# arkiven4/glow-tts

Hardware: AMD Instinct MI355X
Metric: mel_frames_per_sec_train_step (higher is better)
Workload: dtype bf16; 1 GPU; configs/base.json, LJSpeech-shaped synthetic batches, B=32/GPU, T_x<=150, T_y<=800, bf16 GEMMs; batch_per_gpu=32, T_x=150, T_y=800, batches_rotated=8, padded_frames_per_gpu_step=25600, rows_layout=ragged, graphs_captured=6, parallelism=dp1 (utterance-sharded, RCCL gradient all-reduce, fp32 on the wire), launch=one HIP graph per step (one per ragged-row bucket, captured up front)

## Files before the change

### glow-tts_amd/_lib.py

```python
import ctypes
import os

_HERE = os.path.dirname(os.path.abspath(__file__))
LIB_PATH = os.environ.get("GT_LIB") or os.path.join(_HERE, "libglowtts_hip.so")

c_void_p, c_int, c_i64, c_size_t, c_float, c_u32 = (ctypes.c_void_p, ctypes.c_int, ctypes.c_int64,
                                                    ctypes.c_size_t, ctypes.c_float, ctypes.c_uint32)


class Pointer(ctypes.c_void_p):

    @classmethod
    def from_param(cls, v):
        if hasattr(v, "data_ptr"):
            v = v.data_ptr()
        elif isinstance(v, ctypes.Structure):
            return ctypes.byref(v)
        return ctypes.c_void_p.from_param(v)


STATUS = "status"
c_void_p = Pointer

PROTOTYPES = {
# ... 69 lines not shown
    "gt_embedding_fwd": (STATUS, [c_void_p, c_void_p, c_void_p, c_void_p, c_void_p, c_int, c_int, c_int, c_void_p, c_int, c_int, c_int, c_float, c_void_p]),
    "gt_embedding_bwd": (STATUS, [c_void_p, c_void_p, c_void_p, c_void_p, c_int, c_int, c_int, c_void_p, c_int, c_int, c_int, c_float, c_void_p]),
    "gt_rows_add_cond": (STATUS, [c_void_p, c_int, c_void_p, c_int, c_void_p, c_void_p, c_void_p, c_int, c_void_p, c_int,
                                  c_int, c_int, c_int, c_int, c_void_p, c_void_p]),
    "gt_rows_ctx_fill": (STATUS, [c_void_p, c_void_p, c_void_p, c_void_p, c_void_p, c_void_p, c_int, c_int, c_void_p]),
    "gt_step_inputs": (STATUS, [c_void_p, c_void_p]),
    "gt_step_zero": (STATUS, [c_void_p, c_void_p]),
    "gt_rows_utt_sum": (STATUS, [c_void_p, c_int, c_int, c_void_p, c_void_p, c_int, c_int, c_int, c_int, c_int, c_int, c_void_p, c_void_p]),
    "gt_logp_f32": (STATUS, [c_void_p, c_void_p, c_void_p, c_void_p, c_int, c_int, c_int, c_int, c_void_p]),
    "gt_prior_expand": (STATUS, [c_void_p, c_void_p, c_void_p, c_int, c_int, c_int, c_int, c_void_p]),
    "gt_rows_from_bct": (STATUS, [c_void_p, c_int, c_void_p, c_int, c_void_p, c_int, c_int, c_int, c_int, c_int, c_void_p]),
    "gt_bct_from_rows": (STATUS, [c_void_p, c_int, c_void_p, c_int, c_void_p, c_void_p, c_int, c_int, c_int, c_int, c_int, c_void_p]),
    "gt_mle_finish": (STATUS, [c_void_p, c_void_p, c_void_p, c_int, c_int, c_int, c_void_p, c_void_p]),
    "gt_duration_loss_fwd": (STATUS, [c_void_p, c_void_p, c_void_p, c_int, c_int, c_void_p, c_void_p]),
    "gt_duration_loss_bwd": (STATUS, [c_void_p, c_void_p, c_void_p, c_void_p, c_int, c_int, c_void_p, c_void_p]),
    "gt_prior_expand_bwd": (STATUS, [c_void_p, c_void_p, c_void_p, c_int, c_int, c_int, c_int, c_void_p]),
    "gt_mle_sums": (STATUS, [c_void_p, c_void_p, c_void_p, c_void_p, c_size_t, c_void_p]),
    "gt_mle_bwd": (STATUS, [c_void_p, c_void_p, c_void_p, c_void_p, c_void_p, c_void_p, c_void_p, c_size_t, c_void_p, c_void_p, c_int, c_void_p]),
    "gt_mark": (STATUS, [c_void_p, c_void_p]),
    "gt_length_mask": (STATUS, [c_void_p, c_int, c_void_p, c_int, c_int, c_void_p]),
    "gt_wn_layer_fwd": (STATUS, [c_void_p, c_int, c_void_p, c_void_p, c_void_p, c_int, c_void_p, c_int, c_int, c_void_p,
                                 c_void_p, c_int, c_void_p, c_void_p, c_int, c_void_p, c_void_p, c_void_p, c_int,
                                 c_int, c_int, c_int, c_float, c_u32, c_void_p, c_void_p, c_int, c_void_p, c_void_p]),
    "gt_wn_layer_bwd": (STATUS, [c_void_p, c_int, c_void_p, c_void_p, c_int, c_void_p, c_void_p, c_int, c_void_p,
                                 c_void_p, c_int, c_void_p, c_void_p, c_int, c_void_p, c_void_p, c_int, c_int, c_int, c_int, c_float, c_u32,
                                 c_void_p, c_void_p, c_int, c_void_p, c_void_p]),
    "gt_wn_stack_fwd": (STATUS, [c_void_p, c_void_p]),
    "gt_wn_stack_rows_per_workgroup": (c_int, [c_int]),
    "gt_wn_stack_row_blocks": (c_int, [c_int, c_int, c_int]),
    "gt_cond_affine_grads": (STATUS, [c_void_p, c_void_p, c_void_p, c_void_p, c_int, c_void_p, c_void_p, c_void_p, c_int, c_int, c_int, c_void_p]),
# ... 366 lines not shown
```

### glow-tts_amd/csrc/encoder_ops.hip

```cpp
#include <stdlib.h>
#include "common.h"
#include "../../include/glowtts_hip.h"
#include "internal.h"

namespace {

constexpr int HALO = GT_HALO;

struct LnArgs {
  const float* a; const bf16_t* y; int ldy;
  const float* gamma; const float* beta;
  const float* rowmask;
  float* out_f32; bf16_t* out_bf16; int ldo;
  float* mean; float* rstd;
  int R, C; float eps;
  uint32_t din_thresh, din_seed; float din_scale;
  uint32_t dout_thresh, dout_seed; float dout_scale;
  int relu;
  const uint32_t* seed_dev;
};

template <typename T> __device__ __forceinline__ void ln_landed(T& x) { asm volatile("" : "+v"(x)); }

template <bool HAS_A, bool HAS_Y>
// ... 795 lines not shown
                                            const float* __restrict__ g, int B, int Tx, float* __restrict__ dlogw)
{
  const int b = blockIdx.x, lane = threadIdx.x;
  float tot = 0.f;
  for (int i = lane; i < B; i += 64) tot += (float)len[i];
  tot = wave_sum(tot);
  const int n = len[b];
  const float gb = 2.0f * g[b] / tot;
  for (int t = lane; t < Tx; t += 64) {
    const float lw = logw[(size_t)b * Tx + t];
    const float ref = t < n ? __logf(w[(size_t)b * Tx + t] + 1e-8f) : 0.f;
    dlogw[(size_t)b * Tx + t] = gb * (lw - ref);
  }
}

}

#define GT_ST(s) static_cast<hipStream_t>(s)
#define GT_RET() return gt_launch_status(__func__)

static int fill_ln(LnArgs& p, const float* a, const void* y, int ldy, const float* gamma, const float* beta, const float* rowmask,
                   float* out_f32, void* out_bf16, int ldo, float* mean, float* rstd, int R, int C, float eps,
                   float p_in, uint32_t seed_in, float p_out, uint32_t seed_out, int relu, const uint32_t* seed_dev)
{
  if ((!a && !y) || !gamma || !beta || !mean || !rstd || R <= 0 || C <= 0 || C > 256) return GT_E_INVAL;
  if (p_in >= 1.f || p_out >= 1.f) return GT_E_INVAL;
  p.a = a; p.y = static_cast<const bf16_t*>(y); p.ldy = ldy; p.gamma = gamma; p.beta = beta; p.rowmask = rowmask;
  p.out_f32 = out_f32; p.out_bf16 = static_cast<bf16_t*>(out_bf16); p.ldo = ldo; p.mean = mean; p.rstd = rstd;
  p.R = R; p.C = C; p.eps = eps; p.relu = relu; p.seed_dev = seed_dev;
  p.din_seed = seed_in; p.dout_seed = seed_out;
// ... 352 lines not shown
  GT_RET();
}
extern "C" int gt_duration_loss_fwd(const float* logw, const float* w, const int32_t* x_lengths, int B, int Tx, float* l_length, void* stream)
{
  if (!logw || !w || !x_lengths || !l_length || B <= 0 || Tx <= 0) return GT_E_INVAL;
  hipLaunchKernelGGL(gt_duration_loss_fwd_kernel, dim3(B), dim3(64), 0, GT_ST(stream), logw, w, x_lengths, B, Tx, l_length);
  GT_RET();
}
extern "C" int gt_duration_loss_bwd(const float* logw, const float* w, const int32_t* x_lengths, const float* g, int B, int Tx,
                                    float* dlogw, void* stream)
{
  if (!logw || !w || !x_lengths || !g || !dlogw || B <= 0 || Tx <= 0) return GT_E_INVAL;
  hipLaunchKernelGGL(gt_duration_loss_bwd_kernel, dim3(B), dim3(64), 0, GT_ST(stream), logw, w, x_lengths, g, B, Tx, dlogw);
  GT_RET();
}
extern "C" int gt_mle_bwd(const float* z, const float* m, const float* logs, const float* gscale, float* dz, float* dm, float* dlogs,
                          size_t n, const float* gdenom, float* dlogdet, int B, void* stream)
{
  if (!z || !m || !gscale) return GT_E_INVAL;
  if (n == 0) return GT_OK;
  size_t blocks = (n + 255) / 256; if (blocks > 2048) blocks = 2048;
  hipLaunchKernelGGL(gt_mle_bwd_kernel, dim3((unsigned)blocks), dim3(256), 0, GT_ST(stream), z, m, logs, gscale, dz, dm, dlogs, n, gdenom, dlogdet, B);
  GT_RET();
}
```

### glow-tts_amd/monotonic_align.py

```python
import torch

from . import _lib
from ._lib import call

MAS_MAX_TX, MAS_LDS_CAP = 512, 160 * 1024
MAS_LONG_MAX_TX, MAS_LONG_MAX_TY, MAS_LONG_MAX_B = 4096, 32768, 65535

_DT = {torch.float32: _lib.GT_DT_F32, torch.int32: _lib.GT_DT_I32, torch.float16: _lib.GT_DT_F16,
       torch.bfloat16: _lib.GT_DT_BF16, torch.uint8: _lib.GT_DT_U8}


class MASResult:
    __slots__ = ("path", "durations", "frame2token", "status", "workspace")

    def __init__(self, path, durations, frame2token, status, workspace=None):
        self.path, self.durations, self.frame2token, self.status = path, durations, frame2token, status
        self.workspace = workspace


def maximum_path_lengths(value, t_x, t_y, mask=None, out_dtype=None, want_durations=False,
                         want_frame2token=False, validate=False, keep_workspace=False, allow_long=False):
    _lib.require_cuda(value, t_x, t_y, mask)
    if value.dim() != 3:
        raise ValueError("value must be [b, t_x, t_y]")
    out_dtype = out_dtype or value.dtype
    if out_dtype not in _DT:
        raise TypeError(f"unsupported path dtype {out_dtype}")
    v = value.detach()
    if v.dtype != torch.float32:
        v = v.float()
    if v.stride(2) != 1:
        v = v.contiguous()
    B, T_x, T_y = v.shape
    m = None
    if mask is not None:
        m = mask.detach().to(torch.float32).expand_as(v)
        if m.stride() != v.stride():
            m = m.contiguous()
            v = v.contiguous()
    t_x = t_x.to(device=v.device, dtype=torch.int32).contiguous()
    t_y = t_y.to(device=v.device, dtype=torch.int32).contiguous()
    path = torch.empty((B, T_x, T_y), dtype=out_dtype, device=v.device)
    dur = torch.empty((B, T_x), dtype=torch.float32, device=v.device) if want_durations else None
    f2t = torch.empty((B, T_y), dtype=torch.int32, device=v.device) if want_frame2token else None
    status = torch.zeros((1,), dtype=torch.int32, device=v.device) if validate else None
    ws = None
    if B and T_x and T_y:
        args = (v, m, t_x, t_y, path, _DT[out_dtype], dur, f2t, B, T_x, T_y, v.stride(0), v.stride(1))
        if allow_long and not fits_lds_kernel(T_x, T_y):
            if T_x > MAS_LONG_MAX_TX or T_y > MAS_LONG_MAX_TY or B > MAS_LONG_MAX_B:
                raise RuntimeError(f"gt_mas_long_f32: lattice [{B},{T_x},{T_y}] exceeds the kernel's limits (T_x<={MAS_LONG_MAX_TX}, "
                                   f"T_y<={MAS_LONG_MAX_TY}, B<={MAS_LONG_MAX_B})")
            ws_bytes = call.gt_mas_long_workspace_bytes(B, T_x, T_y)
            ws = torch.empty((ws_bytes // 4,), dtype=torch.int32, device=v.device)
            call.gt_mas_long_f32(*args, ws, ws_bytes, status, _lib.current_stream(v.device))
        else:
            ws_bytes = call.gt_mas_workspace_bytes(B, T_x, T_y)
# ... 54 lines not shown
```

### glow-tts_amd/ops.py

```python
import torch

from . import _lib, devstate
from ._lib import call

HALO = 2


def _round_up(x, m):
    return (x + m - 1) // m * m


class _KernelTimer:

    def __init__(self):
        self.tag, self.pairs = None, []

    def enable(self, tag):
        self.tag, self.pairs = tag, []

    def disable(self):
        self.tag = None

    def start(self, tag):
        if self.tag is None or tag != self.tag:
# ... 140 lines not shown

    def __init__(self, ragged=False, row_round=128):
        self.ragged = ragged
        self.row_round = row_round
        self.host_lengths = {}
        self.prebuilt = {}
        self.stamps = None
        self.frame_rows_ragged = True
        self.attn_keep_p = True
        import os
        self.encoder_stream = os.environ.get("GT_ENC_STREAM", "1") != "0"
        self.predictor_branch = os.environ.get("GT_PRED_BRANCH", "1") != "0"
        self.energy_on_main = os.environ.get("GT_ENERGY_MAIN", "1") != "0"
        self.dp_balance = os.environ.get("GT_DP_BALANCE", "1") != "0"
        self.join_predictors = True
        self.front_stream = os.environ.get("GT_FRONT_STREAM", "1") != "0"


DEFAULT_ROWS = RowsConfig()


def rows_add_cond(rc, x, xb, cond, want_f32=True, want_bf16=True):
    src = x if x is not None else xb
    R, C = src.shape
    dev = src.device
    cond = cond.detach().float().contiguous()
    assert cond.shape == (rc.B, C), (cond.shape, rc.B, C)
    out = torch.empty(R, C, dtype=torch.float32, device=dev) if want_f32 else None
    outb = torch.empty(R, C, dtype=torch.bfloat16, device=dev) if want_bf16 else None
    call.gt_rows_add_cond(x, 0 if x is None else x.stride(0), xb, 0 if xb is None else xb.stride(0), cond, rc.rowmask, out, C, outb, C, rc.B, R, C,
# ... 298 lines not shown
```

### glow-tts_amd/text_models.py

```python
import math
import contextlib
import os

import torch
from torch import nn

from . import _lib, devstate, encoder_impl, ops
from ._lib import call
from . import monotonic_align
from .attentions import Encoder
from .modules import ConvP, ConvReluNorm, LayerNorm, _RowsFn, prepare_all
from .ops import HALO, PackedConv, RowsCtx


class _PaddedConv:
    weight_norm = False

    def __init__(self, conv):
        self.conv, self.pc, self.weight, self.bias = conv, None, None, None

    def refresh(self):
        c = self.conv
        dev = c.weight.device
        if self.pc is None or self.pc.fwd.device != dev:
# ... 200 lines not shown
        grads = {}
        d8 = torch.zeros(rc.B, 8, rc.T, dtype=torch.float32, device=rc.device)
        d8[:, 0] = dlogw[:, 0].float()
        dout = rc.to_rows(d8)
        from . import wgrad
        ops.mark("dp bwd begin")
        with wgrad.WgradQueue(rc.device, site=self.dp):
            dxb = encoder_impl.dp_bwd(rc, self.dp, saved, dout, grads, want_dx=self.has_cond)
        ops.mark("dp bwd end")
        return ([ops.cond_grad(rc, dxb)] if self.has_cond else []) + [grads.get(p) for p in self.params]


class _LogpMasFn:

    @staticmethod
    def run(x_m, x_logs, z, x_lengths, y_lengths, mean_only):
        B, C, Tx = x_m.shape
        Ty = z.shape[2]
        dev = z.device
        logp = torch.empty(B, Tx, Ty, dtype=torch.float32, device=dev)
        xm = x_m.detach().float().contiguous()
        xs = None if mean_only else x_logs.detach().float().contiguous()
        zz = z.detach().float().contiguous()
        call.gt_logp_f32(xm, xs, zz, logp, B, C, Tx, Ty, _lib.current_stream(dev))
        r = monotonic_align.maximum_path_lengths(logp, x_lengths.to(torch.int32), y_lengths.to(torch.int32),
                                                 want_durations=True, want_frame2token=True, keep_workspace=True, allow_long=True)
        return logp, r


class _PriorExpandFn(torch.autograd.Function):

    @staticmethod
    def forward(ctx, x_m, f2t, starts):
        B, C, Tx = x_m.shape
        Ty = f2t.shape[1]
        xm = x_m.detach().float().contiguous()
        z_m = torch.empty(B, C, Ty, dtype=torch.float32, device=x_m.device)
        call.gt_prior_expand(xm, f2t, z_m, B, C, Tx, Ty, _lib.current_stream(x_m.device))
        ctx.f2t, ctx.shape = f2t, (B, C, Tx, Ty)
        return z_m

# ... 47 lines not shown
        wc = w.detach().float().contiguous()
        xl = x_lengths.to(torch.int32).contiguous()
        out = torch.empty(B, dtype=torch.float32, device=lw.device)
        call.gt_duration_loss_fwd(lw, wc, xl, B, Tx, out, _lib.current_stream(lw.device))
        ctx.saved = (lw, wc, xl, logw.shape)
        return out

    @staticmethod
    def backward(ctx, g):
        lw, wc, xl, shape = ctx.saved
        B, _, Tx = shape
        gc = g.float().contiguous()
        d = torch.empty(shape, dtype=torch.float32, device=lw.device)
        call.gt_duration_loss_bwd(lw, wc, xl, gc, B, Tx, d, _lib.current_stream(lw.device))
        return d, None, None


def mle_loss(z, m, logs, logdet, mask):
    return _MleLossFn.apply(z, m, logs, logdet, mask)


def _front_stream(dev):
    return devstate.get(dev).stream("front")


def _encoder_stream(dev):
    return devstate.get(dev).stream("encoder")


class FlowGenerator(nn.Module):
# ... 318 lines not shown
                xo, x_m, x_logs, x_mask = self.encoder(x, x_lengths, l=l, g=g, prepared=True)
                ops.mark("enc fwd end")
                if not self.use_sdp and not dp_here:
                    logw = self._predict_logw(g, l)
                    ops.mark("dp fwd end")
        else:
            xo, x_m, x_logs, x_mask = self.encoder(x, x_lengths, l=l, g=g, prepared=True)
        self._deferred = []
        if defer_encoder_backward:
            leaf = x_m.detach().requires_grad_(True)
            self._deferred.append((x_m, leaf)); x_m = leaf
            if not self.mean_only:
                leaf = x_logs.detach().requires_grad_(True)
                self._deferred.append((x_logs, leaf)); x_logs = leaf
        y, y_lengths, y_max_length = self.preprocess(y, y_lengths, y.size(2))
        z_mask = ops.length_mask(y_lengths, y_max_length, x_mask.dtype)
        pitch_norm, energy_norm = self._contour(pitch, y_max_length), self._contour(energy, y_max_length)
        ops.mark("dec fwd begin")
        z, logdet = self.decoder(y, z_mask, g=g, pitch=pitch_norm, energy=energy_norm, prepared=True)
        ops.mark("dec fwd end")
        if fork:
            main.wait_stream(enc_stream)
            ops.mark("fwd joined")
            for t_ in (xo, x_m, x_logs, x_mask, self.encoder._last_rows[1]) + ((logw,) if logw is not None else ()):
                t_.record_stream(main)
            if dp_here:
                logw = self._predict_logw(g, l)
                ops.mark("dp fwd end")
        with torch.no_grad():
            logp, mas = _LogpMasFn.run(x_m, x_logs, z, x_lengths, y_lengths, self.mean_only)
            self._last_mas_path = mas.path
            if path is not None:
                mas = monotonic_align.result_from_path(path.reshape(mas.path.shape).to(mas.path.dtype), x_lengths.to(torch.int32),
                                                       y_lengths.to(torch.int32))
            attn = mas.path.unsqueeze(1)
        ops.mark("mas done")
        w = mas.durations.unsqueeze(1)
        rcx, xb = self.encoder._last_rows
        pfork = fork and self.rows_cfg.predictor_branch and (self.use_sdp or self.use_spp or self.use_sep)
        if pfork:
            enc_stream.wait_stream(main)
            for t_ in (w, mas.frame2token, mas.durations, pitch_norm, energy_norm, z_mask, x_mask, y_lengths):
                if t_ is not None:
                    t_.record_stream(enc_stream)
        with (torch.cuda.stream(enc_stream) if pfork else contextlib.nullcontext()):
            l_length, l_pitch, l_energy, logw = self._predictor_losses(rcx, xb, w, x_mask, x_lengths, z_mask, g, l, logw, noise, mas, y_lengths,
                                                                       y_max_length, pitch_norm, energy_norm,
                                                                       energy_stream=main if (pfork and self.rows_cfg.energy_on_main) else None)
        self._loss_streams = None
        if pfork and self.rows_cfg.join_predictors:
            main.wait_stream(enc_stream)
            for t_ in (l_length, l_pitch, l_energy):
                if t_ is not None:
                    t_.record_stream(main)
        elif pfork:
            self._loss_streams = {"stream": enc_stream, "energy_on_caller": bool(self.rows_cfg.energy_on_main and self.use_spp and self.use_sep)}
        z_m = _PriorExpandFn.apply(x_m, mas.frame2token, mas.workspace)
        z_logs = torch.zeros_like(z_m) if self.mean_only else _PriorExpandFn.apply(x_logs, mas.frame2token, mas.workspace)
        self.last_logp = logp
        return (z, z_m, z_logs, logdet, z_mask), (x_m, x_logs, x_mask), (attn, l_length, l_pitch, l_energy), (None, None, None, None), None

    def _predictor_losses(self, rcx, xb, w, x_mask, x_lengths, z_mask, g, l, logw, noise, mas, y_lengths, y_max_length, pitch_norm, energy_norm,
                          energy_stream=None):
        l_pitch = l_energy = None
        rcf = xf = zsum = ready = None
        if self.use_spp or self.use_sep:
            rcf = ops.make_ctx(y_lengths.to(torch.int32), y_max_length, "f", cfg=self.rows_cfg)
            xf = self._gather_features(rcx, xb, rcf, mas.frame2token)
            zsum = torch.sum(z_mask)
            if energy_stream is not None and xf.is_cuda and self.use_spp and self.use_sep:
                ready = torch.cuda.Event()
                ready.record(torch.cuda.current_stream(xf.device))
        if self.use_sdp:
            pw = self.encoder.proj_w
            w_rows = rcx.to_rows(w.float())[:, 0].contiguous()
            nw = None if noise is None else rcx.to_rows(noise[0].float())
            l_length = pw.nll_rows(rcx, xb, w_rows, pw.cond_vec(g, l), nw) / torch.sum(x_mask)
        else:
            if logw is None:
                logw = self._predict_logw(g, l)
            l_length = _DurationLossFn.apply(logw, w, x_lengths)
        if self.use_spp or self.use_sep:
            if self.use_spp:
                pp = self.proj_pitch
                npz = None if noise is None else rcf.to_rows(noise[1].float())[:, 0].contiguous()
                l_pitch = torch.sum(pp.nll_rows(rcf, xf, rcf.to_rows(pitch_norm.float())[:, 0].contiguous(), pp.cond_vec(g), npz) / zsum)
            if self.use_sep:
                es = energy_stream if ready is not None else None
                if es is not None:
                    es.wait_event(ready)
                    xf.record_stream(es); zsum.record_stream(es)
                with (torch.cuda.stream(es) if es is not None else contextlib.nullcontext()):
                    pe = self.proj_energy
                    nez = None if noise is None else rcf.to_rows(noise[2].float())[:, 0].contiguous()
                    l_energy = torch.sum(pe.nll_rows(rcf, xf, rcf.to_rows(energy_norm.float())[:, 0].contiguous(), pe.cond_vec(g), nez) / zsum)
        return l_length, l_pitch, l_energy, logw
# ... 1 lines not shown
```

### glow-tts_amd/train.py

```python
import json
import math
import os

import contextlib
import torch
import torch.distributed as dist

from . import _lib, models
from ._lib import call

BASE_MODEL = dict(hidden_channels=192, filter_channels=768, filter_channels_dp=256, kernel_size=3, p_dropout=0.1,
                  n_blocks_dec=12, n_layers_enc=6, n_heads=2, p_dropout_dec=0.05, dilation_rate=1, kernel_size_dec=5,
                  n_block_layers=4, n_sqz=2, prenet=True, mean_only=True, hidden_channels_enc=192,
                  hidden_channels_dec=192, window_size=4,
                  use_sdp=False)


def load_model_config(path=None):
    if path and os.path.exists(path):
        with open(path) as f:
            return dict(json.load(f)["model"])
    return dict(BASE_MODEL)


# ... 319 lines not shown
            if len(self.seen) >= self.max_tracked:
                self.seen.clear()
            self.seen[key] = n
            return False
        self.seen.pop(key, None)
        return True


class Trainer:

    WARMUPS = 2

    def __init__(self, model, lr=2e-4, betas=(0.9, 0.98), eps=1e-9, world=1, graph=False, total_steps=None,
                 split_graph=None, ragged=None, max_graphs=8, pad_tx=16, pad_ty=32, kernel_stamps=False, grad_wire="fp32",
                 force_collectives=False, capture_after=2, ty_boundaries=None, row_round=None, early_decoder_adam=True, pack_in_tail=True, split_roots=True,
                 attn_keep_p=None):
        from collections import OrderedDict
        self.model = model
        self.world = world
        self.early_decoder_adam = bool(early_decoder_adam)
        self.pack_in_tail = bool(pack_in_tail)
        self.split_roots = bool(split_roots)
        self._dec_fresh_version = None
        self._head_rest = self._tail_packed = False
        self.graph_mode = bool(graph)
        self.split = bool(split_graph)
        accum = []
        for mod in model.modules():
            kind = type(mod).__name__
            if kind in ("LayerNorm", "ActNorm", "InvConvNear", "Embedding"):
                accum += list(mod.parameters(recurse=False))
            elif kind == "MultiHeadAttention":
                accum += [mod.emb_rel_k, mod.emb_rel_v]
        named = list(model.named_parameters())
        late = lambda n: ".cond_layer." in n or "cond_layer1" in n
        plist = [p for n, p in named if not n.startswith("decoder.")] + [p for n, p in named if n.startswith("decoder.") and late(n)] + \
# ... 26 lines not shown
        self.ty_boundaries = list(ty_boundaries) if ty_boundaries else None
        self.stamps = None
        if kernel_stamps:
            from . import ops
            dec = model.decoder
            per_step = dec.n_blocks * dec.n_layers * (3 if hasattr(dec.flows[2], "wn_pitch") else 1)
            self.stamps = self.cfg.stamps = ops.KernelStamps(next(model.parameters()).device, per_step)

    @property
    def adam_steps(self):
        return int(self.opt.hyper[5].item())

    def _loss(self, outs):
        m = self.model
        (z, z_m, z_logs, logdet, z_mask), _, (attn, l_length, l_pitch, l_energy), _, _ = outs
        l_mle = models.mle_loss(z, z_m, None if m.mean_only else z_logs, logdet, z_mask)
        loss = l_mle + torch.sum(l_length)
        if l_pitch is not None:
            loss = loss + 0.5 * l_pitch
        if l_energy is not None:
            loss = loss + 0.5 * l_energy
        return loss, l_mle

    def _loss_roots(self, outs):
        m = self.model
        ls = getattr(m, "_loss_streams", None)
        if ls is None:
            loss, l_mle = self._loss(outs)
            return [loss], l_mle
        (z, z_m, z_logs, logdet, z_mask), _, (attn, l_length, l_pitch, l_energy), _, _ = outs
        l_mle = models.mle_loss(z, z_m, None if m.mean_only else z_logs, logdet, z_mask)
        here = l_mle
        with torch.cuda.stream(ls["stream"]):
            there = torch.sum(l_length)
            if l_pitch is not None:
                there = there + 0.5 * l_pitch
            if l_energy is not None and not ls["energy_on_caller"]:
                there = there + 0.5 * l_energy
        if l_energy is not None and ls["energy_on_caller"]:
            here = here + 0.5 * l_energy
        return [here, there], l_mle

    def _begin(self, device):
        from . import ops
        if self.stamps is not None:
            self.stamps.begin_step()
        if ops.MARKS is not None:
# ... 28 lines not shown
    def _early_decoder_update(self, params_done):
        done = {id(p) for p in params_done}
        if all(id(p) in done for p in self.buckets.params[self.dec_cov:]) and self.dec_cov_off < self.buckets.total:
            self.opt.step_early(self.dec_cov_off, self.buckets.total)
            if self.pack_in_tail and self.cfg.encoder_stream and hasattr(self.model, "prepare"):
                self.model.prepare(part="decoder")
                self._tail_packed = True
                self._dec_fresh_version = self._param_version()

    def _fwd_bwd(self, ids, t_x, y, t_y, lengths_host=None, cond=None, early_update=False):
        self._begin(ids.device)
        from . import ops
        rows_cfg = getattr(self.model, "rows_cfg", None)
        if rows_cfg is not None:
            rows_cfg.join_predictors = not self.split_roots
        try:
            roots, l_mle = self._loss_roots(self.model(ids, t_x, y, t_y, lengths_host=lengths_host, **(cond or {})))
        finally:
            if rows_cfg is not None:
                rows_cfg.join_predictors = True
        ops.mark("loss")
        dec = getattr(self.model, "decoder", None)
        early = early_update and self.early_decoder_adam and dec is not None and not self.buckets.collect and ids.is_cuda
        if early:
            object.__setattr__(dec, "_gt_after_flush", self._early_decoder_update)
        try:
            if len(roots) == 1:
                roots[0].backward()
            else:
                torch.autograd.backward(roots)
        finally:
            if early:
                object.__setattr__(dec, "_gt_after_flush", None)
        if len(roots) > 1:
            torch.cuda.current_stream().wait_stream(self.model._loss_streams["stream"])
# ... 5 lines not shown
        ops.mark("gradients gathered")
        return loss.detach(), l_mle.detach()

    def _optim(self, device):
        from . import ops
        if self._grad_norm_buf is None:
            self._grad_norm_buf = torch.zeros(1, dtype=torch.float32, device=device)
        self.grad_norm = torch.sqrt(self.opt.step(), out=self._grad_norm_buf)
        ops.mark("optimizer done")
        if self.stamps is not None:
            self.stamps.end_step()
        ops.arena_end(device)

    def _phase1(self, ids, t_x, y, t_y, lengths_host=None, cond=None):
        self._begin(ids.device)
        loss, l_mle = self._loss(self.model(ids, t_x, y, t_y, lengths_host=lengths_host, defer_encoder_backward=True,
                                            **(cond or {})))
        loss.backward()
        self.buckets.gather(self.dec0, None)
        return loss.detach(), l_mle.detach()

    def _phase2(self):
        self.model.backward_encoder()
        self.buckets.gather(0, self.dec0)

    def _step_impl(self, ids, t_x, y, t_y, lengths_host=None, cond=None, collectives=True):
        if not self.split:
            out = self._fwd_bwd(ids, t_x, y, t_y, lengths_host, cond, early_update=True)
            if collectives:
                self.buckets.allreduce()
        else:
            out = self._phase1(ids, t_x, y, t_y, lengths_host, cond)
# ... 210 lines not shown
```

### include/glowtts_hip.h

```cpp
#ifndef GLOWTTS_HIP_H
#define GLOWTTS_HIP_H

#include <stddef.h>
#include <stdint.h>

#ifdef __cplusplus
extern "C" {
#endif

#define GT_OK            0
#define GT_E_INVAL      -1
#define GT_E_UNSUPPORTED -2
#define GT_E_ALIGN      -3
#define GT_E_LAUNCH     -4

#define GT_DT_F32  0
#define GT_DT_I32  1
#define GT_DT_F16  2
#define GT_DT_BF16 3
#define GT_DT_U8   4

#define GT_MAS_ST_TX_GT_TY   1
#define GT_MAS_ST_BAD_LEN    2

// ... 189 lines not shown
int gt_logp_f32(const float* x_m, const float* x_logs, const float* z, float* logp, int B, int C, int Tx, int Ty, void* stream);

int gt_prior_expand(const float* x_m, const int32_t* frame2token, float* z_m, int B, int C, int Tx, int Ty, void* stream);
int gt_prior_expand_bwd(const float* dz_m, const int32_t* frame2token, float* dx_m, int B, int C, int Tx, int Ty, void* stream);

#define GT_MLE_PARTS 2048
int gt_mle_sums(const float* z, const float* m, const float* logs, float* acc2, size_t n, void* stream);
int gt_mle_bwd(const float* z, const float* m, const float* logs, const float* gscale, float* dz, float* dm, float* dlogs,
               size_t n, const float* gdenom, float* dlogdet, int B, void* stream);
int gt_mark(unsigned long long* slot, void* stream);
int gt_length_mask(const void* lengths, int is_int64, float* mask, int B, int T, void* stream);

int gt_mle_finish(const float* acc2, const float* logdet, const float* mask, int n_mask, int B, int C, float* out2, void* stream);
int gt_duration_loss_fwd(const float* logw, const float* w, const int32_t* x_lengths, int B, int Tx, float* l_length, void* stream);
int gt_duration_loss_bwd(const float* logw, const float* w, const int32_t* x_lengths, const float* g, int B, int Tx, float* dlogw, void* stream);

int gt_rows_from_bct(const void* x, int x_f32, void* rows, int rows_f32, const int32_t* row0, int B, int C, int T, int Tp, int R, void* stream);
int gt_bct_from_rows(const void* rows, int rows_f32, void* x, int x_f32, const int32_t* lengths, const int32_t* row0,
                     int B, int C, int T, int Tp, int R, void* stream);

int gt_actnorm_invconv_rev(const float* y, float* x, void* x0_bf16, int ld0, const float* logs, const float* bias,
                           const float* scal, const float* rowmask, int R, int C, void* stream);
int gt_coupling_rev(const float* out, const float* z, float* x, const float* rowmask, int R, int C,
                    int sigmoid_scale, void* stream);

int gt_adamw_flat(float* p, const float* g, float* m, float* v, size_t n, const float* hyper,
                  float* gnorm_sq, void* stream);

typedef struct gt_wn_stack_fwd_args {
  const void* x0;
// ... 264 lines not shown
```

Before: 4.910 million mel-frames/s.

## Fuse prior expansion, MLE loss and duration loss into single align-loss kernels

Adds fused forward, finish and backward kernels that do the prior expansion (frame2token gather), the MLE partial sums and the duration loss in one launch each. The backward scatters dz into dx_m and dx_logs with segmented wave-scans in shared memory instead of a separate prior-expand backward. MAS can now skip materialising the dense path tensor. The aim is to cut launch count and round trips through global memory in the loss stage. The trainer enables it by default and keeps the old path as a fallback.

```diff
diff --git a/glow-tts_amd/_lib.py b/glow-tts_amd/_lib.py
--- a/glow-tts_amd/_lib.py
+++ b/glow-tts_amd/_lib.py
@@ -107,6 +107,9 @@
     "gt_mle_finish": (STATUS, [c_void_p, c_void_p, c_void_p, c_int, c_int, c_int, c_void_p, c_void_p]),
     "gt_duration_loss_fwd": (STATUS, [c_void_p, c_void_p, c_void_p, c_int, c_int, c_void_p, c_void_p]),
     "gt_duration_loss_bwd": (STATUS, [c_void_p, c_void_p, c_void_p, c_void_p, c_int, c_int, c_void_p, c_void_p]),
+    "gt_align_loss_fwd": (STATUS, [c_void_p] * 11 + [c_int, c_int, c_int, c_int, c_void_p]),
+    "gt_align_loss_finish": (STATUS, [c_void_p, c_void_p, c_void_p, c_int, c_void_p, c_int, c_int, c_void_p, c_void_p]),
+    "gt_align_loss_bwd": (STATUS, [c_void_p] * 14 + [c_int, c_int, c_int, c_int, c_void_p]),
     "gt_prior_expand_bwd": (STATUS, [c_void_p, c_void_p, c_void_p, c_int, c_int, c_int, c_int, c_void_p]),
     "gt_mle_sums": (STATUS, [c_void_p, c_void_p, c_void_p, c_void_p, c_size_t, c_void_p]),
     "gt_mle_bwd": (STATUS, [c_void_p, c_void_p, c_void_p, c_void_p, c_void_p, c_void_p, c_void_p, c_size_t, c_void_p, c_void_p, c_int, c_void_p]),
diff --git a/glow-tts_amd/csrc/encoder_ops.hip b/glow-tts_amd/csrc/encoder_ops.hip
--- a/glow-tts_amd/csrc/encoder_ops.hip
+++ b/glow-tts_amd/csrc/encoder_ops.hip
@@ -833,6 +833,179 @@
   }
 }
 
+__global__ __launch_bounds__(256) void gt_align_loss_fwd_kernel(const float* __restrict__ z, const float* __restrict__ xm,
+                                                                const float* __restrict__ xlogs, const int32_t* __restrict__ f2t,
+                                                                const float* __restrict__ logw, const float* __restrict__ w,
+                                                                const int32_t* __restrict__ len, float* __restrict__ zm,
+                                                                float* __restrict__ zlogs, float* __restrict__ acc,
+                                                                float* __restrict__ l_length, int B, int C, int Tx, int Ty)
+{
+  if (blockIdx.x >= GT_MLE_PARTS) {
+    const int b = blockIdx.x - GT_MLE_PARTS, lane = threadIdx.x;
+    if (lane >= 64) return;
+    float tot = 0.f;
+    for (int i = lane; i < B; i += 64) tot += (float)len[i];
+    tot = wave_sum(tot);
+    float a = 0.f;
+    const int n = len[b];
+    for (int t = lane; t < Tx; t += 64) {
+      const float lw = logw[(size_t)b * Tx + t];
+      const float ref = t < n ? __logf(w[(size_t)b * Tx + t] + 1e-8f) : 0.f;
+      const float d = lw - ref;
+      a += d * d;
+    }
+    a = wave_sum(a);
+    if (lane == 0) l_length[b] = a / tot;
+    return;
+  }
+  __shared__ float red[2][4];
+  float a0 = 0.f, a1 = 0.f;
+  const unsigned ty4 = (unsigned)Ty >> 2;
+  const unsigned n4 = (unsigned)B * C * ty4;
+  for (unsigned i = blockIdx.x * 256 + threadIdx.x; i < n4; i += GT_MLE_PARTS * 256) {
+    const unsigned bc = i / ty4, j4 = i - bc * ty4, b = bc / C;
+    const int4 t = reinterpret_cast<const int4*>(f2t)[(size_t)b * ty4 + j4];
+    const bool v0 = (unsigned)t.x < (unsigned)Tx, v1 = (unsigned)t.y < (unsigned)Tx, v2 = (unsigned)t.z < (unsigned)Tx,
+               v3 = (unsigned)t.w < (unsigned)Tx;
+    const float* xr = xm + (size_t)bc * Tx;
+    const float4 zz = reinterpret_cast<const float4*>(z)[i];
+    const float4 mm = make_float4(v0 ? xr[t.x] : 0.f, v1 ? xr[t.y] : 0.f, v2 ? xr[t.z] : 0.f, v3 ? xr[t.w] : 0.f);
+    float4 ll = make_float4(0.f, 0.f, 0.f, 0.f);
+    if (xlogs) {
+      const float* sr = xlogs + (size_t)bc * Tx;
+      ll = make_float4(v0 ? sr[t.x] : 0.f, v1 ? sr[t.y] : 0.f, v2 ? sr[t.z] : 0.f, v3 ? sr[t.w] : 0.f);
+      reinterpret_cast<float4*>(zlogs)[i] = ll;
+    }
+    reinterpret_cast<float4*>(zm)[i] = mm;
+    const float d0 = zz.x - mm.x, d1 = zz.y - mm.y, d2 = zz.z - mm.z, d3 = zz.w - mm.w;
+    a0 += ll.x + ll.y + ll.z + ll.w;
+    a1 += __expf(-2.0f * ll.x) * d0 * d0 + __expf(-2.0f * ll.y) * d1 * d1 + __expf(-2.0f * ll.z) * d2 * d2 + __expf(-2.0f * ll.w) * d3 * d3;
+  }
+  a0 = wave_sum(a0); a1 = wave_sum(a1);
+  if ((threadIdx.x & 63) == 0) { red[0][threadIdx.x >> 6] = a0; red[1][threadIdx.x >> 6] = a1; }
+  __syncthreads();
+  if (threadIdx.x == 0) {
+    acc[2 * blockIdx.x] = red[0][0] + red[0][1] + red[0][2] + red[0][3];
+    acc[2 * blockIdx.x + 1] = red[1][0] + red[1][1] + red[1][2] + red[1][3];
+  }
+}
+
+__global__ __launch_bounds__(1024) void gt_align_loss_finish_kernel(const float* __restrict__ acc, const float* __restrict__ logdet,
+                                                                    const float* __restrict__ mask, int n_mask,
+                                                                    const float* __restrict__ l_length, int B, int C, float* __restrict__ out)
+{
+  __shared__ float red[2][16];
+  __shared__ float red2[2];
+  {
+    float p0 = 0.f, p1 = 0.f;
+    for (int i = threadIdx.x; i < GT_MLE_PARTS; i += 1024) { const float2 v = reinterpret_cast<const float2*>(acc)[i]; p0 += v.x; p1 += v.y; }
+    p0 = wave_sum(p0); p1 = wave_sum(p1);
+    if ((threadIdx.x & 63) == 0) { red[0][threadIdx.x >> 6] = p0; red[1][threadIdx.x >> 6] = p1; }
+    __syncthreads();
+    if (threadIdx.x == 0) {
+      p0 = 0.f; p1 = 0.f;
+#pragma unroll
+      for (int i = 0; i < 16; ++i) { p0 += red[0][i]; p1 += red[1][i]; }
+      red2[0] = p0; red2[1] = p1;
+    }
+    __syncthreads();
+  }
+  float sl = 0.f, sn = 0.f;
+  for (int b = threadIdx.x; b < B; b += 1024) sl += logdet[b];
+  const int n4 = ((reinterpret_cast<uintptr_t>(mask) & 15) == 0) ? n_mask >> 2 : 0;
+  for (int i = threadIdx.x; i < n4; i += 1024) { const float4 v = reinterpret_cast<const float4*>(mask)[i]; sn += (v.x + v.y) + (v.z + v.w); }
+  for (int i = (n4 << 2) + threadIdx.x; i < n_mask; i += 1024) sn += mask[i];
+  sl = wave_sum(sl); sn = wave_sum(sn);
+  if ((threadIdx.x & 63) == 0) { red[0][threadIdx.x >> 6] = sl; red[1][threadIdx.x >> 6] = sn; }
+  float ll = 0.f;
+  if (l_length && threadIdx.x < 64) {
+    int nt = 1;
+    while (nt * 2 <= B && nt < 64) nt <<= 1;
+    if ((int)threadIdx.x < nt)
+      for (int i = threadIdx.x; i < B; i += nt) ll += l_length[i];
+    for (int off = 1; off < nt; off <<= 1) ll += __shfl_down(ll, off);
+  }
+  __syncthreads();
+  if (threadIdx.x == 0) {
+    sl = 0.f; sn = 0.f;
+#pragma unroll
+    for (int i = 0; i < 16; ++i) { sl += red[0][i]; sn += red[1][i]; }
+    const float denom = sn * (float)C;
+    const float mle = (red2[0] + 0.5f * red2[1] - sl) / denom + 0.91893853320467274f;
+    out[0] = mle;
+    out[1] = denom;
+    out[2] = ll;
+    out[3] = mle + ll;
+  }
+}
+
+template <bool LOGS>
+__global__ __launch_bounds__(256) void gt_align_loss_bwd_kernel(const float* __restrict__ z, const float* __restrict__ zm,
+                                                                const float* __restrict__ zlogs, const int32_t* __restrict__ f2t,
+                                                                const float* __restrict__ logw, const float* __restrict__ w,
+                                                                const int32_t* __restrict__ len, const float* __restrict__ gscale,
+                                                                const float* __restrict__ gdenom, float* __restrict__ dz,
+                                                                float* __restrict__ dxm, float* __restrict__ dxlogs,
+                                                                float* __restrict__ dlogdet, float* __restrict__ dlogw,
+                                                                int B, int C, int Tx, int Ty, int row_blocks)
+{
+  __shared__ float acc[LOGS ? 2 : 1][4][512];
+  if ((int)blockIdx.x >= row_blocks) {
+    const int e = blockIdx.x - row_blocks;
+    if (e == 0) {
+      const float g = *gscale / *gdenom;
+      for (int b = threadIdx.x; b < B; b += 256) dlogdet[b] = -g;
+      return;
+    }
+    const int b = e - 1, lane = threadIdx.x;
+    if (lane >= 64) return;
+    float tot = 0.f;
+    for (int i = lane; i < B; i += 64) tot += (float)len[i];
+    tot = wave_sum(tot);
+    const int n = len[b];
+    const float gb = 2.0f * *gscale / tot;
+    for (int t = lane; t < Tx; t += 64) {
+      const float lw = logw[(size_t)b * Tx + t];
+      const float ref = t < n ? __logf(w[(size_t)b * Tx + t] + 1e-8f) : 0.f;
+      dlogw[(size_t)b * Tx + t] = gb * (lw - ref);
+    }
+    return;
+  }
+  const int lane = threadIdx.x & 63, wave = threadIdx.x >> 6;
+  const int bc = blockIdx.x * 4 + wave;
+  if (bc >= B * C) return;
+  const int b = bc / C;
+  const float g = *gscale / *gdenom;
+  float* am = acc[0][wave];
+  float* as = acc[LOGS ? 1 : 0][wave];
+  for (int i = lane; i < Tx; i += 64) { am[i] = 0.f; if (LOGS) as[i] = 0.f; }
+  for (int j0 = 0; j0 < Ty; j0 += 64) {
+    const int j = j0 + lane;
+    int t = -1; float vm = 0.f, vs = 0.f;
+    if (j < Ty) {
+      const size_t i = (size_t)bc * Ty + j;
+      t = f2t[(size_t)b * Ty + j];
+      const float l = LOGS ? zlogs[i] : 0.f, e = __expf(-2.0f * l), d = z[i] - zm[i];
+      const float v = g * e * d;
+      dz[i] = v;
+      vm = -v;
+      if (LOGS) vs = g * (1.0f - e * d * d);
+    }
+#pragma unroll
+    for (int off = 1; off < 64; off <<= 1) {
+      const float um = __shfl_up(vm, off), us = LOGS ? __shfl_up(vs, off) : 0.f;
+      const int tt = __shfl_up(t, off);
+      if (lane >= off && tt == t) { vm += um; if (LOGS) vs += us; }
+    }
+    const int tn = __shfl_down(t, 1);
+    if (t >= 0 && t < Tx && (lane == 63 || tn != t)) { am[t] += vm; if (LOGS) as[t] += vs; }
+  }
+  for (int i = lane; i < Tx; i += 64) {
+    dxm[(size_t)bc * Tx + i] = am[i];
+    if (LOGS) dxlogs[(size_t)bc * Tx + i] = as[i];
+  }
+}
+
 }
 
 #define GT_ST(s) static_cast<hipStream_t>(s)
@@ -1215,6 +1388,49 @@
   hipLaunchKernelGGL(gt_duration_loss_bwd_kernel, dim3(B), dim3(64), 0, GT_ST(stream), logw, w, x_lengths, g, B, Tx, dlogw);
   GT_RET();
 }
+extern "C" int gt_align_loss_fwd(const float* z, const float* x_m, const float* x_logs, const int32_t* frame2token, const float* logw,
+                                 const float* w, const int32_t* x_lengths, float* z_m, float* z_logs, float* acc2, float* l_length,
+                                 int B, int C, int Tx, int Ty, void* stream)
+{
+  if (!z || !x_m || !frame2token || !z_m || !acc2 || (x_logs && !z_logs) || B <= 0 || C <= 0 || Tx <= 0 || Ty <= 0) return GT_E_INVAL;
+  if ((logw != nullptr) != (w != nullptr) || (logw && (!x_lengths || !l_length))) return GT_E_INVAL;
+  if (Tx > 512) return GT_E_UNSUPPORTED;
+  if ((size_t)B * C * Ty > 0x7fffffffu) return GT_E_UNSUPPORTED;
+  if (Ty & 3) return GT_E_ALIGN;
+  if (((uintptr_t)z | (uintptr_t)z_m | (uintptr_t)z_logs | (uintptr_t)frame2token) & 15) return GT_E_ALIGN;
+  if ((uintptr_t)acc2 & 7) return GT_E_ALIGN;
+  hipLaunchKernelGGL(gt_align_loss_fwd_kernel, dim3(GT_MLE_PARTS + (logw ? B : 0)), dim3(256), 0, GT_ST(stream), z, x_m, x_logs, frame2token,
+                     logw, w, x_lengths, z_m, z_logs, acc2, l_length, B, C, Tx, Ty);
+  GT_RET();
+}
+extern "C" int gt_align_loss_finish(const float* acc2, const float* logdet, const float* mask, int n_mask, const float* l_length, int B, int C,
+                                    float* out4, void* stream)
+{
+  if (!acc2 || !logdet || !mask || !out4 || B <= 0 || C <= 0 || n_mask <= 0) return GT_E_INVAL;
+  if ((uintptr_t)acc2 & 7) return GT_E_ALIGN;
+  hipLaunchKernelGGL(gt_align_loss_finish_kernel, dim3(1), dim3(1024), 0, GT_ST(stream), acc2, logdet, mask, n_mask, l_length, B, C, out4);
+  GT_RET();
+}
+extern "C" int gt_align_loss_bwd(const float* z, const float* z_m, const float* z_logs, const int32_t* frame2token, const float* logw,
+                                 const float* w, const int32_t* x_lengths, const float* gscale, const float* gdenom, float* dz, float* dx_m,
+                                 float* dx_logs, float* dlogdet, float* dlogw, int B, int C, int Tx, int Ty, void* stream)
+{
+  if (!z || !z_m || !frame2token || !gscale || !gdenom || !dz || !dx_m || !dlogdet || (z_logs && !dx_logs) || B <= 0 || C <= 0 || Tx <= 0 ||
+      Ty <= 0)
+    return GT_E_INVAL;
+  if ((logw != nullptr) != (w != nullptr) || (logw && (!x_lengths || !dlogw))) return GT_E_INVAL;
+  if (Tx > 512) return GT_E_UNSUPPORTED;
+  if ((size_t)B * C * Ty > 0x7fffffffu) return GT_E_UNSUPPORTED;
+  const int row_blocks = (int)(((size_t)B * C + 3) / 4);
+  const dim3 grid(row_blocks + 1 + (logw ? B : 0));
+  if (z_logs)
+    hipLaunchKernelGGL(gt_align_loss_bwd_kernel<true>, grid, dim3(256), 0, GT_ST(stream), z, z_m, z_logs, frame2token, logw, w, x_lengths, gscale,
+                       gdenom, dz, dx_m, dx_logs, dlogdet, dlogw, B, C, Tx, Ty, row_blocks);
+  else
+    hipLaunchKernelGGL(gt_align_loss_bwd_kernel<false>, grid, dim3(256), 0, GT_ST(stream), z, z_m, z_logs, frame2token, logw, w, x_lengths, gscale,
+                       gdenom, dz, dx_m, dx_logs, dlogdet, dlogw, B, C, Tx, Ty, row_blocks);
+  GT_RET();
+}
 extern "C" int gt_mle_bwd(const float* z, const float* m, const float* logs, const float* gscale, float* dz, float* dm, float* dlogs,
                           size_t n, const float* gdenom, float* dlogdet, int B, void* stream)
 {
diff --git a/glow-tts_amd/monotonic_align.py b/glow-tts_amd/monotonic_align.py
--- a/glow-tts_amd/monotonic_align.py
+++ b/glow-tts_amd/monotonic_align.py
@@ -19,7 +19,7 @@
 
 
 def maximum_path_lengths(value, t_x, t_y, mask=None, out_dtype=None, want_durations=False,
-                         want_frame2token=False, validate=False, keep_workspace=False, allow_long=False):
+                         want_frame2token=False, validate=False, keep_workspace=False, allow_long=False, want_path=True):
     _lib.require_cuda(value, t_x, t_y, mask)
     if value.dim() != 3:
         raise ValueError("value must be [b, t_x, t_y]")
@@ -40,7 +40,7 @@
             v = v.contiguous()
     t_x = t_x.to(device=v.device, dtype=torch.int32).contiguous()
     t_y = t_y.to(device=v.device, dtype=torch.int32).contiguous()
-    path = torch.empty((B, T_x, T_y), dtype=out_dtype, device=v.device)
+    path = torch.empty((B, T_x, T_y), dtype=out_dtype, device=v.device) if want_path else None
     dur = torch.empty((B, T_x), dtype=torch.float32, device=v.device) if want_durations else None
     f2t = torch.empty((B, T_y), dtype=torch.int32, device=v.device) if want_frame2token else None
     status = torch.zeros((1,), dtype=torch.int32, device=v.device) if validate else None
diff --git a/glow-tts_amd/ops.py b/glow-tts_amd/ops.py
--- a/glow-tts_amd/ops.py
+++ b/glow-tts_amd/ops.py
@@ -178,6 +178,7 @@
         self.energy_on_main = os.environ.get("GT_ENERGY_MAIN", "1") != "0"
         self.dp_balance = os.environ.get("GT_DP_BALANCE", "1") != "0"
         self.join_predictors = True
+        self.fused_align_loss = False
         self.front_stream = os.environ.get("GT_FRONT_STREAM", "1") != "0"
 
 
diff --git a/glow-tts_amd/text_models.py b/glow-tts_amd/text_models.py
--- a/glow-tts_amd/text_models.py
+++ b/glow-tts_amd/text_models.py
@@ -238,7 +238,7 @@
 class _LogpMasFn:
 
     @staticmethod
-    def run(x_m, x_logs, z, x_lengths, y_lengths, mean_only):
+    def run(x_m, x_logs, z, x_lengths, y_lengths, mean_only, want_path=True):
         B, C, Tx = x_m.shape
         Ty = z.shape[2]
         dev = z.device
@@ -248,7 +248,8 @@
         zz = z.detach().float().contiguous()
         call.gt_logp_f32(xm, xs, zz, logp, B, C, Tx, Ty, _lib.current_stream(dev))
         r = monotonic_align.maximum_path_lengths(logp, x_lengths.to(torch.int32), y_lengths.to(torch.int32),
-                                                 want_durations=True, want_frame2token=True, keep_workspace=True, allow_long=True)
+                                                 want_durations=True, want_frame2token=True, keep_workspace=True, allow_long=True,
+                                                 want_path=want_path)
         return logp, r
 
 
@@ -326,6 +327,52 @@
         d = torch.empty(shape, dtype=torch.float32, device=lw.device)
         call.gt_duration_loss_bwd(lw, wc, xl, gc, B, Tx, d, _lib.current_stream(lw.device))
         return d, None, None
+
+
+class _AlignLossFn(torch.autograd.Function):
+
+    @staticmethod
+    def forward(ctx, z, x_m, x_logs, logdet, logw, w, f2t, x_len32, mask):
+        dev = z.device
+        B, C, Tx = x_m.shape
+        Ty = z.shape[2]
+        st = _lib.current_stream(dev)
+        new = lambda *shape: torch.empty(*shape, dtype=torch.float32, device=dev)
+        zc, xm = z.detach().float().contiguous(), x_m.detach().float().contiguous()
+        xs = None if x_logs is None else x_logs.detach().float().contiguous()
+        lw = None if logw is None else logw.detach().float().contiguous()
+        wc = None if logw is None else w.detach().float().contiguous()
+        z_m = new(B, C, Ty)
+        z_logs = None if xs is None else new(B, C, Ty)
+        l_length = None if lw is None else new(B)
+        acc = new(2 * _lib.MLE_PARTS)
+        call.gt_align_loss_fwd(zc, xm, xs, f2t, lw, wc, x_len32, z_m, z_logs, acc, l_length, B, C, Tx, Ty, st)
+        ld = logdet.detach().float().contiguous()
+        mk = mask.detach().float().contiguous()
+        out = new(4)
+        call.gt_align_loss_finish(acc, ld, mk, mk.numel(), l_length, ld.numel(), C, out, st)
+        ctx.saved = (zc, z_m, z_logs, f2t, lw, wc, x_len32, out, (B, C, Tx, Ty), logdet.shape, None if logw is None else logw.shape)
+        res = (out[3], out[0], z_m, z_logs, l_length)
+        ctx.mark_non_differentiable(*[t for t in res[1:] if t is not None])
+        ctx.set_materialize_grads(False)
+        return res
+
+    @staticmethod
+    def backward(ctx, g, *unused):
+        if g is None:
+            return (None,) * 9
+        zc, z_m, z_logs, f2t, lw, wc, x_len32, out, (B, C, Tx, Ty), ld_shape, lw_shape = ctx.saved
+        dev = zc.device
+        new = lambda *shape: torch.empty(*shape, dtype=torch.float32, device=dev)
+        gs = g.float().reshape(1).contiguous()
+        dz = torch.empty_like(zc)
+        dx_m = new(B, C, Tx)
+        dx_logs = None if z_logs is None else new(B, C, Tx)
+        dlogdet = new(ld_shape)
+        dlogw = None if lw is None else new(lw_shape)
+        call.gt_align_loss_bwd(zc, z_m, z_logs, f2t, lw, wc, x_len32, gs, out[1:].data_ptr(), dz, dx_m, dx_logs, dlogdet, dlogw,
+                               B, C, Tx, Ty, _lib.current_stream(dev))
+        return dz, dx_m, dx_logs, dlogdet, dlogw, None, None, None, None
 
 
 def mle_loss(z, m, logs, logdet, mask):
@@ -674,6 +721,9 @@
                 leaf = x_logs.detach().requires_grad_(True)
                 self._deferred.append((x_logs, leaf)); x_logs = leaf
         y, y_lengths, y_max_length = self.preprocess(y, y_lengths, y.size(2))
+        self._fused_loss = None
+        fused = bool(self.rows_cfg.fused_align_loss) and path is None and x.is_cuda and x.shape[1] <= 512 and y_max_length % 4 == 0
+        y_len32 = y_lengths.to(torch.int32) if fused else None
         z_mask = ops.length_mask(y_lengths, y_max_length, x_mask.dtype)
         pitch_norm, energy_norm = self._contour(pitch, y_max_length), self._contour(energy, y_max_length)
         ops.mark("dec fwd begin")
@@ -687,17 +737,21 @@
             if dp_here:
                 logw = self._predict_logw(g, l)
                 ops.mark("dp fwd end")
+        rcx, xb = self.encoder._last_rows
         with torch.no_grad():
-            logp, mas = _LogpMasFn.run(x_m, x_logs, z, x_lengths, y_lengths, self.mean_only)
+            if fused:
+                logp, mas = _LogpMasFn.run(x_m, x_logs, z, rcx.lengths, y_len32, self.mean_only, want_path=False)
+            else:
+                logp, mas = _LogpMasFn.run(x_m, x_logs, z, x_lengths, y_lengths, self.mean_only)
             self._last_mas_path = mas.path
             if path is not None:
                 mas = monotonic_align.result_from_path(path.reshape(mas.path.shape).to(mas.path.dtype), x_lengths.to(torch.int32),
                                                        y_lengths.to(torch.int32))
-            attn = mas.path.unsqueeze(1)
+            attn = None if mas.path is None else mas.path.unsqueeze(1)
         ops.mark("mas done")
         w = mas.durations.unsqueeze(1)
-        rcx, xb = self.encoder._last_rows
         pfork = fork and self.rows_cfg.predictor_branch and (self.use_sdp or self.use_spp or self.use_sep)
+        dur_fused = fused and not self.use_sdp and not pfork
         if pfork:
             enc_stream.wait_stream(main)
             for t_ in (w, mas.frame2token, mas.durations, pitch_norm, energy_norm, z_mask, x_mask, y_lengths):
@@ -706,7 +760,8 @@
         with (torch.cuda.stream(enc_stream) if pfork else contextlib.nullcontext()):
             l_length, l_pitch, l_energy, logw = self._predictor_losses(rcx, xb, w, x_mask, x_lengths, z_mask, g, l, logw, noise, mas, y_lengths,
                                                                        y_max_length, pitch_norm, energy_norm,
-                                                                       energy_stream=main if (pfork and self.rows_cfg.energy_on_main) else None)
+                                                                       energy_stream=main if (pfork and self.rows_cfg.energy_on_main) else None,
+                                                                       skip_duration_loss=dur_fused)
         self._loss_streams = None
         if pfork and self.rows_cfg.join_predictors:
             main.wait_stream(enc_stream)
@@ -715,13 +770,20 @@
                     t_.record_stream(main)
         elif pfork:
             self._loss_streams = {"stream": enc_stream, "energy_on_caller": bool(self.rows_cfg.energy_on_main and self.use_spp and self.use_sep)}
+        self.last_logp = logp
+        if fused:
+            total, l_mle, z_m, z_logs, ll = _AlignLossFn.apply(z, x_m, None if self.mean_only else x_logs, logdet, logw if dur_fused else None,
+                                                               w if dur_fused else None, mas.frame2token, rcx.lengths, z_mask)
+            if dur_fused:
+                l_length = ll
+            self._fused_loss = (total, l_mle, dur_fused)
+            return (z, z_m, z_logs, logdet, z_mask), (x_m, x_logs, x_mask), (attn, l_length, l_pitch, l_energy), (None, None, None, None), None
         z_m = _PriorExpandFn.apply(x_m, mas.frame2token, mas.workspace)
         z_logs = torch.zeros_like(z_m) if self.mean_only else _PriorExpandFn.apply(x_logs, mas.frame2token, mas.workspace)
-        self.last_logp = logp
         return (z, z_m, z_logs, logdet, z_mask), (x_m, x_logs, x_mask), (attn, l_length, l_pitch, l_energy), (None, None, None, None), None
 
     def _predictor_losses(self, rcx, xb, w, x_mask, x_lengths, z_mask, g, l, logw, noise, mas, y_lengths, y_max_length, pitch_norm, energy_norm,
-                          energy_stream=None):
+                          energy_stream=None, skip_duration_loss=False):
         l_pitch = l_energy = None
         rcf = xf = zsum = ready = None
         if self.use_spp or self.use_sep:
@@ -739,7 +801,7 @@
         else:
             if logw is None:
                 logw = self._predict_logw(g, l)
-            l_length = _DurationLossFn.apply(logw, w, x_lengths)
+            l_length = None if skip_duration_loss else _DurationLossFn.apply(logw, w, x_lengths)
         if self.use_spp or self.use_sep:
             if self.use_spp:
                 pp = self.proj_pitch
diff --git a/glow-tts_amd/train.py b/glow-tts_amd/train.py
--- a/glow-tts_amd/train.py
+++ b/glow-tts_amd/train.py
@@ -357,12 +357,13 @@
     def __init__(self, model, lr=2e-4, betas=(0.9, 0.98), eps=1e-9, world=1, graph=False, total_steps=None,
                  split_graph=None, ragged=None, max_graphs=8, pad_tx=16, pad_ty=32, kernel_stamps=False, grad_wire="fp32",
                  force_collectives=False, capture_after=2, ty_boundaries=None, row_round=None, early_decoder_adam=True, pack_in_tail=True, split_roots=True,
-                 attn_keep_p=None):
+                 attn_keep_p=None, fused_align_loss=True):
         from collections import OrderedDict
         self.model = model
         self.world = world
         self.early_decoder_adam = bool(early_decoder_adam)
         self.pack_in_tail = bool(pack_in_tail)
+        self.fused_align_loss = bool(fused_align_loss)
         self.split_roots = bool(split_roots)
         self._dec_fresh_version = None
         self._head_rest = self._tail_packed = False
@@ -419,8 +420,13 @@
     def _loss(self, outs):
         m = self.model
         (z, z_m, z_logs, logdet, z_mask), _, (attn, l_length, l_pitch, l_energy), _, _ = outs
-        l_mle = models.mle_loss(z, z_m, None if m.mean_only else z_logs, logdet, z_mask)
-        loss = l_mle + torch.sum(l_length)
+        fl = m.__dict__.pop("_fused_loss", None)
+        if fl is not None:
+            l_mle = fl[1]
+            loss = fl[0] if fl[2] else fl[0] + torch.sum(l_length)
+        else:
+            l_mle = models.mle_loss(z, z_m, None if m.mean_only else z_logs, logdet, z_mask)
+            loss = l_mle + torch.sum(l_length)
         if l_pitch is not None:
             loss = loss + 0.5 * l_pitch
         if l_energy is not None:
@@ -434,8 +440,11 @@
             loss, l_mle = self._loss(outs)
             return [loss], l_mle
         (z, z_m, z_logs, logdet, z_mask), _, (attn, l_length, l_pitch, l_energy), _, _ = outs
-        l_mle = models.mle_loss(z, z_m, None if m.mean_only else z_logs, logdet, z_mask)
-        here = l_mle
+        fl = m.__dict__.pop("_fused_loss", None)
+        if fl is not None:
+            here, l_mle = fl[0], fl[1]
+        else:
+            here = l_mle = models.mle_loss(z, z_m, None if m.mean_only else z_logs, logdet, z_mask)
         with torch.cuda.stream(ls["stream"]):
             there = torch.sum(l_length)
             if l_pitch is not None:
@@ -494,11 +503,13 @@
         rows_cfg = getattr(self.model, "rows_cfg", None)
         if rows_cfg is not None:
             rows_cfg.join_predictors = not self.split_roots
+            rows_cfg.fused_align_loss = self.fused_align_loss
         try:
             roots, l_mle = self._loss_roots(self.model(ids, t_x, y, t_y, lengths_host=lengths_host, **(cond or {})))
         finally:
             if rows_cfg is not None:
                 rows_cfg.join_predictors = True
+                rows_cfg.fused_align_loss = False
         ops.mark("loss")
         dec = getattr(self.model, "decoder", None)
         early = early_update and self.early_decoder_adam and dec is not None and not self.buckets.collect and ids.is_cuda
@@ -534,8 +545,15 @@
 
     def _phase1(self, ids, t_x, y, t_y, lengths_host=None, cond=None):
         self._begin(ids.device)
-        loss, l_mle = self._loss(self.model(ids, t_x, y, t_y, lengths_host=lengths_host, defer_encoder_backward=True,
-                                            **(cond or {})))
+        rows_cfg = getattr(self.model, "rows_cfg", None)
+        if rows_cfg is not None:
+            rows_cfg.fused_align_loss = self.fused_align_loss
+        try:
+            loss, l_mle = self._loss(self.model(ids, t_x, y, t_y, lengths_host=lengths_host, defer_encoder_backward=True,
+                                                **(cond or {})))
+        finally:
+            if rows_cfg is not None:
+                rows_cfg.fused_align_loss = False
         loss.backward()
         self.buckets.gather(self.dec0, None)
         return loss.detach(), l_mle.detach()
diff --git a/include/glowtts_hip.h b/include/glowtts_hip.h
--- a/include/glowtts_hip.h
+++ b/include/glowtts_hip.h
@@ -227,6 +227,15 @@
 int gt_mle_finish(const float* acc2, const float* logdet, const float* mask, int n_mask, int B, int C, float* out2, void* stream);
 int gt_duration_loss_fwd(const float* logw, const float* w, const int32_t* x_lengths, int B, int Tx, float* l_length, void* stream);
 int gt_duration_loss_bwd(const float* logw, const float* w, const int32_t* x_lengths, const float* g, int B, int Tx, float* dlogw, void* stream);
+
+int gt_align_loss_fwd(const float* z, const float* x_m, const float* x_logs, const int32_t* frame2token, const float* logw, const float* w,
+                      const int32_t* x_lengths, float* z_m, float* z_logs, float* acc2, float* l_length, int B, int C, int Tx, int Ty,
+                      void* stream);
+int gt_align_loss_finish(const float* acc2, const float* logdet, const float* mask, int n_mask, const float* l_length, int B, int C,
+                         float* out4, void* stream);
+int gt_align_loss_bwd(const float* z, const float* z_m, const float* z_logs, const int32_t* frame2token, const float* logw, const float* w,
+                      const int32_t* x_lengths, const float* gscale, const float* gdenom, float* dz, float* dx_m, float* dx_logs,
+                      float* dlogdet, float* dlogw, int B, int C, int Tx, int Ty, void* stream);
 
 int gt_rows_from_bct(const void* x, int x_f32, void* rows, int rows_f32, const int32_t* row0, int B, int C, int T, int Tp, int R, void* stream);
 int gt_bct_from_rows(const void* rows, int rows_f32, void* x, int x_f32, const int32_t* lengths, const int32_t* row0,
```

Measured after the change: 4.987 million mel-frames/s, median of 6. +1.6%, better.
